# datavizweb/async-rl-tensorflow

Measured on AMD Instinct MI355X. Metric: env-steps/sec (whole node), Pong-v0 84×84×4, 1/2/4/8 MI355X + CPU ref, higher is better.
Workload: dtype fp32; 1 GPU; Pong-v0, 256 envs batched per MI355X, n-step=5, A3C conv net (nips trunk); frames=M1: raw RGB 210x160x3 + screen, game=Pong-v0, trunk=nips, head=feed-forward, env=device, envs_per_gpu=256, n_step=5, action_size=6, algo=a3c, parallelism=dp1, hipgraph=False

## Files before the change

async-rl-tensorflow_amd/csrc/gemm.h:

```cpp
#pragma once
#include "a3c_common.h"
#include "../../include/a3c_hip.h"



enum { EPI_STORE = 0, EPI_BIAS_RELU = 1, EPI_BIAS = 2, EPI_MASK = 3, EPI_MASKBITS = 4 };

struct GemmArgs {
  const float* A; int64_t lda;
  const float* B; int64_t ldb;
  float* C; int64_t ldc;
  int M, N, K;
  int epi;
  const float* bias;
  const float* mask; int64_t ldm;
  float* slab;
  int nsplit;
  int kchunk;
  float* colsum;
  int defer_reduce;
  int xcd;
  int max_wgs;
  int big;
  int wg_split;
  const uint32_t* maskbits;
};

int a3c_gemm(bool a_kcontig, bool b_ncontig, GemmArgs g, hipStream_t s, int* nsplit_eff = nullptr);
int a3c_gemm3(GemmArgs& g0, GemmArgs& g1, GemmArgs& g2, hipStream_t s);
int a3c_gemm_reduce(const GemmArgs& g, hipStream_t s);
int a3c_gemm_plan_split(int M, int N, int K, int target_blocks);

inline int a3c_gemm_effective_split(int K, int nsplit) {
  if (K < 1) return 1;
  int ktiles = (K + 15) / 16;
  if (nsplit < 1) nsplit = 1;
  int per = (ktiles + nsplit - 1) / nsplit;
  return (ktiles + per - 1) / per;
}
```

async-rl-tensorflow_amd/csrc/gemm.hip:

```cpp
#include <cstdlib>
#include "gemm.h"

#define BM 64
#define BN 64
#define BK 16
#define PAD 4

template <bool A_KC, bool B_NC>
__device__ inline void gemm_tile(const GemmArgs& g, int bx, int by, int bz, float (&As)[BK][BM + PAD],
                                 float (&Bs)[BK][BN + PAD]) {
  const int tid = threadIdx.x, lane = tid & 63, wid = tid >> 6;
  const int wm = wid >> 1, wn = wid & 1;
  const int m0 = by * BM, n0 = bx * BN;
  const int ks = bz;
  const int kbeg = ks * g.kchunk;
  const int kend = min(g.K, kbeg + g.kchunk);
  const bool do_colsum = g.colsum != nullptr && by == 0;

  int a_r, a_c, b_r, b_c;
  if (A_KC) { a_r = tid >> 2; a_c = (tid & 3) * 4; }
  else      { a_r = tid >> 4; a_c = (tid & 15) * 4; }
  if (B_NC) { b_r = tid >> 4; b_c = (tid & 15) * 4; }
  else      { b_r = tid >> 2; b_c = (tid & 3) * 4; }

  auto load_a = [&](int k0) -> f32x4 {
    f32x4 v = {0.f, 0.f, 0.f, 0.f};
    if (A_KC) {
      int m = m0 + a_r, k = k0 + a_c;
      if (m < g.M && k < kend) v = *(const f32x4*)(g.A + (int64_t)m * g.lda + k);
    } else {
      int k = k0 + a_r, m = m0 + a_c;
      if (k < kend && m < g.M) v = *(const f32x4*)(g.A + (int64_t)k * g.lda + m);
    }
    return v;
  };
  auto load_b = [&](int k0) -> f32x4 {
    f32x4 v = {0.f, 0.f, 0.f, 0.f};
    if (B_NC) {
      int k = k0 + b_r, n = n0 + b_c;
      if (k < kend && n < g.N) v = *(const f32x4*)(g.B + (int64_t)k * g.ldb + n);
    } else {
      int n = n0 + b_r, k = k0 + b_c;
      if (n < g.N && k < kend) v = *(const f32x4*)(g.B + (int64_t)n * g.ldb + k);
    }
    return v;
  };
  auto store_a = [&](f32x4 v) {
    if (A_KC) { As[a_c][a_r] = v[0]; As[a_c + 1][a_r] = v[1]; As[a_c + 2][a_r] = v[2]; As[a_c + 3][a_r] = v[3]; }
    else      { *(f32x4*)&As[a_r][a_c] = v; }
  };
  auto store_b = [&](f32x4 v) {
    if (B_NC) { *(f32x4*)&Bs[b_r][b_c] = v; }
    else      { Bs[b_c][b_r] = v[0]; Bs[b_c + 1][b_r] = v[1]; Bs[b_c + 2][b_r] = v[2]; Bs[b_c + 3][b_r] = v[3]; }
  };

  f32x16 acc = {};
  float csum = 0.f;
  f32x4 ra = load_a(kbeg), rb = load_b(kbeg);
  for (int k0 = kbeg; k0 < kend; k0 += BK) {
    __syncthreads();
    store_a(ra);
    store_b(rb);
    __syncthreads();
    if (k0 + BK < kend) { ra = load_a(k0 + BK); rb = load_b(k0 + BK); }
    if (do_colsum && tid < BN) {
#pragma unroll
      for (int k = 0; k < BK; ++k) csum += Bs[k][tid];
    }
    const int kh = lane >> 5, c = lane & 31;
#pragma unroll
    for (int kk = 0; kk < BK / 2; ++kk) {
      float a = As[2 * kk + kh][wm * 32 + c];
      float b = Bs[2 * kk + kh][wn * 32 + c];
      acc = __builtin_amdgcn_mfma_f32_32x32x2f32(a, b, acc, 0, 0, 0);
    }
  }

  const int col = n0 + wn * 32 + (lane & 31);
  if (g.nsplit > 1) {
    float* out = g.slab + (int64_t)ks * g.M * g.N;
#pragma unroll
    for (int r = 0; r < 16; ++r) {
      int row = m0 + wm * 32 + (r & 3) + 8 * (r >> 2) + 4 * (lane >> 5);
      if (row < g.M && col < g.N) ST_WT_G(out[(int64_t)row * g.N + col], acc[r]);
    }
  } else {
#pragma unroll
    for (int r = 0; r < 16; ++r) {
      int row = m0 + wm * 32 + (r & 3) + 8 * (r >> 2) + 4 * (lane >> 5);
      if (row < g.M && col < g.N) {
        float v = acc[r];
        if (g.epi == EPI_BIAS_RELU) v = fmaxf(v + g.bias[col], 0.f);
        else if (g.epi == EPI_BIAS) v = v + g.bias[col];
        else if (g.epi == EPI_MASK) v = g.mask[(int64_t)row * g.ldm + col] > 0.f ? v : 0.f;
#ifndef A3C_NO_MASKBITS
      else if (g.epi == EPI_MASKBITS) v = (g.maskbits[(int64_t)row * g.ldm + (col >> 5)] >> (col & 31)) & 1u ? v : 0.f;
#endif
        ST_WT_G(g.C[(int64_t)row * g.ldc + col], v);
      }
    }
  }
  if (do_colsum && tid < BN && n0 + tid < g.N) g.colsum[(int64_t)ks * g.N + n0 + tid] = csum;
}

template <bool A_KC, bool B_NC, int KS>
__global__ void __launch_bounds__(256 * KS) k_gemm_f32_wks(GemmArgs g) {
  WGLOG(5);
  __shared__ __attribute__((aligned(16))) float As[KS][BK][BM + PAD];
  __shared__ __attribute__((aligned(16))) float Bs[KS][BK][BN + PAD];
  const int grp = threadIdx.x >> 8, tid = threadIdx.x & 255, lane = tid & 63, wid = tid >> 6;
  const int wm = wid >> 1, wn = wid & 1;
  int bx = blockIdx.x, by = blockIdx.y;
  if (g.xcd == 1) {
    const int gx = (g.N + BN - 1) / BN, gy = (g.M + BM - 1) / BM;
    const int id = blockIdx.x, slot = id >> 3;
    by = 8 * (slot / gx) + (id & 7);
    bx = slot % gx;
    if (by >= gy) return;
  }
  const int m0 = by * BM, n0 = bx * BN;
  const int ktiles = (g.K + BK - 1) / BK, per = (ktiles + KS - 1) / KS;
  const int kbeg = grp * per * BK, kend = min(g.K, kbeg + per * BK);
  const bool do_colsum = g.colsum != nullptr && by == 0;
  int a_r, a_c, b_r, b_c;
  if (A_KC) { a_r = tid >> 2; a_c = (tid & 3) * 4; } else { a_r = tid >> 4; a_c = (tid & 15) * 4; }
  if (B_NC) { b_r = tid >> 4; b_c = (tid & 15) * 4; } else { b_r = tid >> 2; b_c = (tid & 3) * 4; }
  auto load_a = [&](int k0) -> f32x4 {
    f32x4 v = {0.f, 0.f, 0.f, 0.f};
    if (A_KC) {
      int m = m0 + a_r, k = k0 + a_c;
      if (m < g.M && k < kend) v = *(const f32x4*)(g.A + (int64_t)m * g.lda + k);
    } else {
      int k = k0 + a_r, m = m0 + a_c;
      if (k < kend && m < g.M) v = *(const f32x4*)(g.A + (int64_t)k * g.lda + m);
    }
    return v;
  };
  auto load_b = [&](int k0) -> f32x4 {
    f32x4 v = {0.f, 0.f, 0.f, 0.f};
    if (B_NC) {
      int k = k0 + b_r, n = n0 + b_c;
      if (k < kend && n < g.N) v = *(const f32x4*)(g.B + (int64_t)k * g.ldb + n);
    } else {
      int n = n0 + b_r, k = k0 + b_c;
      if (n < g.N && k < kend) v = *(const f32x4*)(g.B + (int64_t)n * g.ldb + k);
    }
    return v;
  };
  float (&as)[BK][BM + PAD] = As[grp];
  float (&bs)[BK][BN + PAD] = Bs[grp];
  f32x16 acc = {};
  float csum = 0.f;
  f32x4 ra = load_a(kbeg), rb = load_b(kbeg);
  for (int it = 0; it < per; ++it) {
    const int k0 = kbeg + it * BK;
    __syncthreads();
    if (A_KC) { as[a_c][a_r] = ra[0]; as[a_c + 1][a_r] = ra[1]; as[a_c + 2][a_r] = ra[2]; as[a_c + 3][a_r] = ra[3]; }
    else      { *(f32x4*)&as[a_r][a_c] = ra; }
    if (B_NC) { *(f32x4*)&bs[b_r][b_c] = rb; }
    else      { bs[b_c][b_r] = rb[0]; bs[b_c + 1][b_r] = rb[1]; bs[b_c + 2][b_r] = rb[2]; bs[b_c + 3][b_r] = rb[3]; }
    __syncthreads();
    if (it + 1 < per) { ra = load_a(k0 + BK); rb = load_b(k0 + BK); }
    if (do_colsum && tid < BN) {
#pragma unroll
      for (int k = 0; k < BK; ++k) csum += bs[k][tid];
    }
    const int kh = lane >> 5, c = lane & 31;
#pragma unroll
    for (int kk = 0; kk < BK / 2; ++kk)
      acc = __builtin_amdgcn_mfma_f32_32x32x2f32(as[2 * kk + kh][wm * 32 + c], bs[2 * kk + kh][wn * 32 + c], acc, 0, 0, 0);
  }
  static_assert(KS * BK * (BM + PAD) >= 16 * 256 + BN, "fold buffer");
  float* fold = &As[0][0][0];
  for (int q = 1; q < KS; ++q) {
    __syncthreads();
    if (grp == q) {
#pragma unroll
      for (int r = 0; r < 16; ++r) fold[r * 256 + tid] = acc[r];
      if (do_colsum && tid < BN) fold[16 * 256 + tid] = csum;
    }
    __syncthreads();
    if (grp == 0) {
#pragma unroll
      for (int r = 0; r < 16; ++r) acc[r] += fold[r * 256 + tid];
      if (do_colsum && tid < BN) csum += fold[16 * 256 + tid];
    }
  }
  if (grp != 0) return;
  const int col = n0 + wn * 32 + (lane & 31);
#pragma unroll
  for (int r = 0; r < 16; ++r) {
    const int row = m0 + wm * 32 + (r & 3) + 8 * (r >> 2) + 4 * (lane >> 5);
    if (row < g.M && col < g.N) {
      float v = acc[r];
      if (g.epi == EPI_BIAS_RELU) v = fmaxf(v + g.bias[col], 0.f);
      else if (g.epi == EPI_BIAS) v = v + g.bias[col];
      else if (g.epi == EPI_MASK) v = g.mask[(int64_t)row * g.ldm + col] > 0.f ? v : 0.f;
#ifndef A3C_NO_MASKBITS
      else if (g.epi == EPI_MASKBITS) v = (g.maskbits[(int64_t)row * g.ldm + (col >> 5)] >> (col & 31)) & 1u ? v : 0.f;
#endif
      ST_WT_G(g.C[(int64_t)row * g.ldc + col], v);
    }
  }
  if (do_colsum && tid < BN && n0 + tid < g.N) g.colsum[n0 + tid] = csum;
}

template <bool A_KC, bool B_NC>
__global__ void __launch_bounds__(256) k_gemm_f32_big(GemmArgs g) {
  WGLOG(5);
  constexpr int TM = 128, TN = 128;
  __shared__ __attribute__((aligned(16))) float As[BK][TM + PAD];
  __shared__ __attribute__((aligned(16))) float Bs[BK][TN + PAD];
  const int tid = threadIdx.x, lane = tid & 63, wid = tid >> 6;
  const int wm = wid >> 1, wn = wid & 1;
  const int m0 = blockIdx.y * TM, n0 = blockIdx.x * TN;
  const int ks = blockIdx.z;
  const int kbeg = ks * g.kchunk;
  const int kend = min(g.K, kbeg + g.kchunk);
  const bool do_colsum = g.colsum != nullptr && blockIdx.y == 0;
  auto a_rc = [&](int u, int& r, int& c) {
    if (A_KC) { r = (tid >> 2) + 64 * u; c = (tid & 3) * 4; }
    else      { r = (tid >> 5) + 8 * u; c = (tid & 31) * 4; }
  };
  auto b_rc = [&](int u, int& r, int& c) {
    if (B_NC) { r = (tid >> 5) + 8 * u; c = (tid & 31) * 4; }
    else      { r = (tid >> 2) + 64 * u; c = (tid & 3) * 4; }
  };
  auto load_a = [&](int k0, int u) -> f32x4 {
    f32x4 v = {0.f, 0.f, 0.f, 0.f};
    int r, c;
    a_rc(u, r, c);
    if (A_KC) {
      const int m = m0 + r, k = k0 + c;
      if (m < g.M && k < kend) v = *(const f32x4*)(g.A + (int64_t)m * g.lda + k);
    } else {
      const int k = k0 + r, m = m0 + c;
      if (k < kend && m < g.M) v = *(const f32x4*)(g.A + (int64_t)k * g.lda + m);
    }
    return v;
  };
  auto load_b = [&](int k0, int u) -> f32x4 {
    f32x4 v = {0.f, 0.f, 0.f, 0.f};
    int r, c;
    b_rc(u, r, c);
    if (B_NC) {
      const int k = k0 + r, n = n0 + c;
      if (k < kend && n < g.N) v = *(const f32x4*)(g.B + (int64_t)k * g.ldb + n);
    } else {
      const int n = n0 + r, k = k0 + c;
      if (n < g.N && k < kend) v = *(const f32x4*)(g.B + (int64_t)n * g.ldb + k);
    }
    return v;
  };
  auto store_a = [&](f32x4 v, int u) {
    int r, c;
    a_rc(u, r, c);
    if (A_KC) { As[c][r] = v[0]; As[c + 1][r] = v[1]; As[c + 2][r] = v[2]; As[c + 3][r] = v[3]; }
    else      { *(f32x4*)&As[r][c] = v; }
  };
  auto store_b = [&](f32x4 v, int u) {
    int r, c;
    b_rc(u, r, c);
    if (B_NC) { *(f32x4*)&Bs[r][c] = v; }
    else      { Bs[c][r] = v[0]; Bs[c + 1][r] = v[1]; Bs[c + 2][r] = v[2]; Bs[c + 3][r] = v[3]; }
  };
  f32x16 acc[2][2] = {};
  float csum = 0.f;
  f32x4 ra0 = load_a(kbeg, 0), ra1 = load_a(kbeg, 1), rb0 = load_b(kbeg, 0), rb1 = load_b(kbeg, 1);
  for (int k0 = kbeg; k0 < kend; k0 += BK) {
    __syncthreads();
    store_a(ra0, 0); store_a(ra1, 1);
    store_b(rb0, 0); store_b(rb1, 1);
    __syncthreads();
    if (k0 + BK < kend) {
      ra0 = load_a(k0 + BK, 0); ra1 = load_a(k0 + BK, 1);
      rb0 = load_b(k0 + BK, 0); rb1 = load_b(k0 + BK, 1);
    }
    if (do_colsum && tid < TN) {
#pragma unroll
      for (int k = 0; k < BK; ++k) csum += Bs[k][tid];
    }
    const int kh = lane >> 5, c = lane & 31;
#pragma unroll
    for (int kk = 0; kk < BK / 2; ++kk) {
      const float a0 = As[2 * kk + kh][wm * 64 + c], a1 = As[2 * kk + kh][wm * 64 + 32 + c];
      const float b0 = Bs[2 * kk + kh][wn * 64 + c], b1 = Bs[2 * kk + kh][wn * 64 + 32 + c];
      acc[0][0] = __builtin_amdgcn_mfma_f32_32x32x2f32(a0, b0, acc[0][0], 0, 0, 0);
      acc[0][1] = __builtin_amdgcn_mfma_f32_32x32x2f32(a0, b1, acc[0][1], 0, 0, 0);
      acc[1][0] = __builtin_amdgcn_mfma_f32_32x32x2f32(a1, b0, acc[1][0], 0, 0, 0);
      acc[1][1] = __builtin_amdgcn_mfma_f32_32x32x2f32(a1, b1, acc[1][1], 0, 0, 0);
    }
  }
#pragma unroll
  for (int i = 0; i < 2; ++i)
#pragma unroll
    for (int j = 0; j < 2; ++j) {
      const int col = n0 + wn * 64 + 32 * j + (lane & 31);
#pragma unroll
      for (int r = 0; r < 16; ++r) {
        const int row = m0 + wm * 64 + 32 * i + (r & 3) + 8 * (r >> 2) + 4 * (lane >> 5);
        if (row >= g.M || col >= g.N) continue;
        float v = acc[i][j][r];
        if (g.nsplit > 1) {
          ST_WT_G(g.slab[(int64_t)ks * g.M * g.N + (int64_t)row * g.N + col], v);
        } else {
          if (g.epi == EPI_BIAS_RELU) v = fmaxf(v + g.bias[col], 0.f);
          else if (g.epi == EPI_BIAS) v = v + g.bias[col];
          else if (g.epi == EPI_MASK) v = g.mask[(int64_t)row * g.ldm + col] > 0.f ? v : 0.f;
#ifndef A3C_NO_MASKBITS
      else if (g.epi == EPI_MASKBITS) v = (g.maskbits[(int64_t)row * g.ldm + (col >> 5)] >> (col & 31)) & 1u ? v : 0.f;
#endif
          ST_WT_G(g.C[(int64_t)row * g.ldc + col], v);
        }
      }
    }
  if (do_colsum && tid < TN && n0 + tid < g.N) g.colsum[(int64_t)ks * g.N + n0 + tid] = csum;
}

template <bool A_KC, bool B_NC>
__device__ inline void gemm_tile_id(const GemmArgs& g, int id, float (&As)[BK][BM + PAD], float (&Bs)[BK][BN + PAD]) {
  const int gx = (g.N + BN - 1) / BN, gy = (g.M + BM - 1) / BM;
  gemm_tile<A_KC, B_NC>(g, id % gx, (id / gx) % gy, id / (gx * gy), As, Bs);
}

template <bool A_KC, bool B_NC>
__global__ void __launch_bounds__(256) k_gemm_f32(GemmArgs g) {
  WGLOG(5);
  __shared__ __attribute__((aligned(16))) float As[BK][BM + PAD];
  __shared__ __attribute__((aligned(16))) float Bs[BK][BN + PAD];
  gemm_tile<A_KC, B_NC>(g, blockIdx.x, blockIdx.y, blockIdx.z, As, Bs);
}

template <bool A_KC, bool B_NC>
__global__ void __launch_bounds__(256) k_gemm_f32_x(GemmArgs g, int G, int J) {
  WGLOG(5);
  __shared__ __attribute__((aligned(16))) float As[BK][BM + PAD];
  __shared__ __attribute__((aligned(16))) float Bs[BK][BN + PAD];
  const int id = blockIdx.x, slot = id >> 3;
  const int grp = 8 * (slot / J) + (id & 7), j = slot % J;
  if (grp >= G) return;
  const int gx = (g.N + BN - 1) / BN, gy = (g.M + BM - 1) / BM;
  if (g.xcd == 1) gemm_tile<A_KC, B_NC>(g, j, grp % gy, grp / gy, As, Bs);
  else gemm_tile<A_KC, B_NC>(g, grp % gx, j, grp / gx, As, Bs);
}

template <bool A_KC, bool B_NC>
__global__ void __launch_bounds__(256) k_gemm_f32_p(GemmArgs g, int nb) {
  WGLOG(5);
  __shared__ __attribute__((aligned(16))) float As[BK][BM + PAD];
  __shared__ __attribute__((aligned(16))) float Bs[BK][BN + PAD];
  for (int id = blockIdx.x; id < nb; id += gridDim.x) gemm_tile_id<A_KC, B_NC>(g, id, As, Bs);
}

template <bool A_KC, bool B_NC>
__global__ void __launch_bounds__(256) k_gemm_f32_xp(GemmArgs g, int G, int J, int nid) {
  WGLOG(5);
  __shared__ __attribute__((aligned(16))) float As[BK][BM + PAD];
  __shared__ __attribute__((aligned(16))) float Bs[BK][BN + PAD];
  const int gx = (g.N + BN - 1) / BN, gy = (g.M + BM - 1) / BM;
  for (int id = blockIdx.x; id < nid; id += gridDim.x) {
    const int slot = id >> 3;
    const int grp = 8 * (slot / J) + (id & 7), j = slot % J;
    if (grp >= G) continue;
    if (g.xcd == 1) gemm_tile<A_KC, B_NC>(g, j, grp % gy, grp / gy, As, Bs);
    else gemm_tile<A_KC, B_NC>(g, grp % gx, j, grp / gx, As, Bs);
  }
}

__global__ void __launch_bounds__(256) k_gemm_multi(GemmArgs g0, GemmArgs g1, GemmArgs g2, int nb0, int nb1) {
  WGLOG(5);
  __shared__ __attribute__((aligned(16))) float As[BK][BM + PAD];
  __shared__ __attribute__((aligned(16))) float Bs[BK][BN + PAD];
  const int id = blockIdx.x;
  if (id < nb0) gemm_tile_id<false, true>(g0, id, As, Bs);
  else if (id < nb0 + nb1) gemm_tile_id<false, true>(g1, id - nb0, As, Bs);
  else gemm_tile_id<true, false>(g2, id - nb0 - nb1, As, Bs);
}

__global__ void k_reduce_slabs(const float* __restrict__ slab, int nsplit, int M, int N,
                               float* __restrict__ C, int64_t ldc, int epi,
                               const float* __restrict__ bias, const float* __restrict__ mask,
                               int64_t ldm, const uint32_t* __restrict__ maskbits) {
  WGLOG(8);
  int64_t i = (int64_t)blockIdx.x * blockDim.x + threadIdx.x;
  int64_t total = (int64_t)M * N;
  if (i >= total) return;
  float v = sum_strided(slab + i, nsplit, total);
  int row = (int)(i / N), col = (int)(i - (int64_t)row * N);
  if (epi == EPI_BIAS_RELU) v = fmaxf(v + bias[col], 0.f);
  else if (epi == EPI_BIAS) v = v + bias[col];
  else if (epi == EPI_MASK) v = mask[(int64_t)row * ldm + col] > 0.f ? v : 0.f;
#ifndef A3C_NO_MASKBITS
  else if (epi == EPI_MASKBITS) v = (maskbits[(int64_t)row * ldm + (col >> 5)] >> (col & 31)) & 1u ? v : 0.f;
#endif
  ST_WT_C(C[(int64_t)row * ldc + col], v);
}

int a3c_gemm_plan_split(int M, int N, int K, int target_blocks) {
  int tiles = ((M + BM - 1) / BM) * ((N + BN - 1) / BN);
  int ktiles = (K + BK - 1) / BK;
  int split = target_blocks / (tiles > 0 ? tiles : 1);
  if (split < 1) split = 1;
  if (split > ktiles) split = ktiles;
  if (split > 32) split = 32;
  return split;
}

static int gemm_setup(bool a_kc, bool b_nc, GemmArgs& g) {
  if (g.K < 1) return a3c_set_error(A3C_ERR_INVALID, "a3c_gemm", "K < 1");
  if (((a_kc || !b_nc) && (g.K & 3)) || (g.lda & 3) || (g.ldb & 3) ||
      (((uintptr_t)g.A | (uintptr_t)g.B) & 15) || (a_kc ? 0 : (g.M & 3)) || (b_nc ? (g.N & 3) : 0))
    return a3c_set_error(A3C_ERR_INVALID, "a3c_gemm", "unaligned operands (need 16-B alignment, dims %4)");
  if (g.nsplit < 1) g.nsplit = 1;
  const int ktiles = (g.K + BK - 1) / BK;
  const int per = (ktiles + g.nsplit - 1) / g.nsplit;
  g.kchunk = per * BK;
  g.nsplit = (ktiles + per - 1) / per;
  if (g.nsplit > 1 && !g.slab) return a3c_set_error(A3C_ERR_INVALID, "a3c_gemm", "split-K needs a slab");
  return 0;
}

static void gemm_reduce(const GemmArgs& g, hipStream_t s) {
  const int64_t total = (int64_t)g.M * g.N;
  hipLaunchKernelGGL(k_reduce_slabs, dim3((unsigned)((total + 255) / 256)), dim3(256), 0, s,
                     g.slab, g.nsplit, g.M, g.N, g.C, g.ldc, g.epi, g.bias, g.mask, g.ldm, g.maskbits);
}

int a3c_gemm3(GemmArgs& g0, GemmArgs& g1, GemmArgs& g2, hipStream_t s) {
  if (g0.M <= 0 || g0.N <= 0 || g1.M <= 0 || g1.N <= 0 || g2.M <= 0 || g2.N <= 0)
    return a3c_set_error(A3C_ERR_INVALID, "a3c_gemm3", "empty GEMM");
  int rc = gemm_setup(false, true, g0);
  if (!rc) rc = gemm_setup(false, true, g1);
  if (!rc) rc = gemm_setup(true, false, g2);
  if (rc) return rc;
  auto blocks = [](const GemmArgs& g) {
    return ((g.N + BN - 1) / BN) * ((g.M + BM - 1) / BM) * g.nsplit;
  };
  const int nb0 = blocks(g0), nb1 = blocks(g1), nb2 = blocks(g2);
  hipLaunchKernelGGL(k_gemm_multi, dim3((unsigned)(nb0 + nb1 + nb2)), dim3(256), 0, s, g0, g1, g2, nb0, nb1);
  A3C_CHECK(hipGetLastError());
  return 0;
}

int a3c_gemm_reduce(const GemmArgs& g, hipStream_t s) {
  if (g.nsplit > 1) {
    gemm_reduce(g, s);
    A3C_CHECK(hipGetLastError());
  }
  return 0;
}

int a3c_gemm(bool a_kc, bool b_nc, GemmArgs g, hipStream_t s, int* nsplit_eff) {
  if (g.M <= 0 || g.N <= 0) return 0;
  if (g.wg_split == 4) {
    g.nsplit = 1;
    int rc = gemm_setup(a_kc, b_nc, g);
    if (rc) return rc;
    if (nsplit_eff) *nsplit_eff = g.nsplit;
    const int gx = (g.N + BN - 1) / BN, gy = (g.M + BM - 1) / BM;
    const dim3 grid = g.xcd == 1 ? dim3((unsigned)(8 * ((gy + 7) / 8) * gx)) : dim3(gx, gy, 1);
    if (g.xcd != 0 && g.xcd != 1) return a3c_set_error(A3C_ERR_INVALID, "a3c_gemm", "wg_split: xcd 0 or 1");
    if (a_kc && b_nc) hipLaunchKernelGGL((k_gemm_f32_wks<true, true, 4>), grid, dim3(1024), 0, s, g);
    else if (a_kc && !b_nc) hipLaunchKernelGGL((k_gemm_f32_wks<true, false, 4>), grid, dim3(1024), 0, s, g);
    else if (!a_kc && b_nc) hipLaunchKernelGGL((k_gemm_f32_wks<false, true, 4>), grid, dim3(1024), 0, s, g);
    else hipLaunchKernelGGL((k_gemm_f32_wks<false, false, 4>), grid, dim3(1024), 0, s, g);
    A3C_CHECK(hipGetLastError());
    return 0;
  }
  if (g.wg_split > 1) return a3c_set_error(A3C_ERR_INVALID, "a3c_gemm", "wg_split: 4 only");
  int rc = gemm_setup(a_kc, b_nc, g);
  if (rc) return rc;
  if (nsplit_eff) *nsplit_eff = g.nsplit;
  dim3 grid((g.N + BN - 1) / BN, (g.M + BM - 1) / BM, g.nsplit);
  const int nb = (int)(grid.x * grid.y * grid.z);
  if (g.big) {
    const dim3 gb((g.N + 127) / 128, (g.M + 127) / 128, g.nsplit);
    if (a_kc && b_nc) hipLaunchKernelGGL((k_gemm_f32_big<true, true>), gb, dim3(256), 0, s, g);
    else if (a_kc && !b_nc) hipLaunchKernelGGL((k_gemm_f32_big<true, false>), gb, dim3(256), 0, s, g);
    else if (!a_kc && b_nc) hipLaunchKernelGGL((k_gemm_f32_big<false, true>), gb, dim3(256), 0, s, g);
    else hipLaunchKernelGGL((k_gemm_f32_big<false, false>), gb, dim3(256), 0, s, g);
    A3C_CHECK(hipGetLastError());
    return g.defer_reduce ? 0 : a3c_gemm_reduce(g, s);
  }
  if (g.xcd) {
    const int G = g.xcd == 1 ? (int)(grid.y * grid.z) : (int)(grid.x * grid.z);
    const int J = g.xcd == 1 ? (int)grid.x : (int)grid.y;
    const int nid = 8 * ((G + 7) / 8) * J;
    if (g.max_wgs > 0 && nid > g.max_wgs) {
      const dim3 gp((unsigned)(8 * ((g.max_wgs + 7) / 8)));
      if (a_kc && b_nc) hipLaunchKernelGGL((k_gemm_f32_xp<true, true>), gp, dim3(256), 0, s, g, G, J, nid);
      else if (a_kc && !b_nc) hipLaunchKernelGGL((k_gemm_f32_xp<true, false>), gp, dim3(256), 0, s, g, G, J, nid);
      else if (!a_kc && b_nc) hipLaunchKernelGGL((k_gemm_f32_xp<false, true>), gp, dim3(256), 0, s, g, G, J, nid);
      else hipLaunchKernelGGL((k_gemm_f32_xp<false, false>), gp, dim3(256), 0, s, g, G, J, nid);
      A3C_CHECK(hipGetLastError());
      return g.defer_reduce ? 0 : a3c_gemm_reduce(g, s);
    }
    const dim3 g1((unsigned)nid);
    if (a_kc && b_nc) hipLaunchKernelGGL((k_gemm_f32_x<true, true>), g1, dim3(256), 0, s, g, G, J);
    else if (a_kc && !b_nc) hipLaunchKernelGGL((k_gemm_f32_x<true, false>), g1, dim3(256), 0, s, g, G, J);
    else if (!a_kc && b_nc) hipLaunchKernelGGL((k_gemm_f32_x<false, true>), g1, dim3(256), 0, s, g, G, J);
    else hipLaunchKernelGGL((k_gemm_f32_x<false, false>), g1, dim3(256), 0, s, g, G, J);
    A3C_CHECK(hipGetLastError());
    return g.defer_reduce ? 0 : a3c_gemm_reduce(g, s);
  }
  if (g.max_wgs > 0 && nb > g.max_wgs) {
    const dim3 gp((unsigned)g.max_wgs);
    if (a_kc && b_nc) hipLaunchKernelGGL((k_gemm_f32_p<true, true>), gp, dim3(256), 0, s, g, nb);
    else if (a_kc && !b_nc) hipLaunchKernelGGL((k_gemm_f32_p<true, false>), gp, dim3(256), 0, s, g, nb);
    else if (!a_kc && b_nc) hipLaunchKernelGGL((k_gemm_f32_p<false, true>), gp, dim3(256), 0, s, g, nb);
    else hipLaunchKernelGGL((k_gemm_f32_p<false, false>), gp, dim3(256), 0, s, g, nb);
    A3C_CHECK(hipGetLastError());
    return g.defer_reduce ? 0 : a3c_gemm_reduce(g, s);
  }
  if (a_kc && b_nc) hipLaunchKernelGGL((k_gemm_f32<true, true>), grid, dim3(256), 0, s, g);
  else if (a_kc && !b_nc) hipLaunchKernelGGL((k_gemm_f32<true, false>), grid, dim3(256), 0, s, g);
  else if (!a_kc && b_nc) hipLaunchKernelGGL((k_gemm_f32<false, true>), grid, dim3(256), 0, s, g);
  else hipLaunchKernelGGL((k_gemm_f32<false, false>), grid, dim3(256), 0, s, g);
  A3C_CHECK(hipGetLastError());
  return g.defer_reduce ? 0 : a3c_gemm_reduce(g, s);
}

static int64_t slab_bytes(int M, int N, int split) {
  return split > 1 ? (int64_t)split * M * N * (int64_t)sizeof(float) : 0;
}

static int gemm_desc_args(const char* what, const a3c_gemm_desc* d, void* ws, int64_t ws_bytes, GemmArgs& g) {
  auto bad = [&](const char* why) { return a3c_set_error(A3C_ERR_INVALID, what, why); };
  auto mis = [](const void* p, uintptr_t a) { return ((uintptr_t)p & (a - 1)) != 0; };
  if (!d) return bad("desc is NULL");
  if (!d->A || !d->B || !d->C) return bad("A, B or C is NULL");
  if (d->M < 1 || d->N < 1) return bad("M < 1 or N < 1");
  if (d->K < 1) return bad("K < 1");
  if (d->nsplit < 1) return bad("nsplit < 1");
  if (d->epi < A3C_GEMM_STORE || d->epi > A3C_GEMM_MASKBITS) return bad("unknown epi");
  if ((d->epi == A3C_GEMM_BIAS_RELU || d->epi == A3C_GEMM_BIAS) && !d->bias) return bad("epi needs bias");
  if (d->epi == A3C_GEMM_MASK && !d->mask) return bad("epi needs mask");
  if (d->epi == A3C_GEMM_MASKBITS && !d->maskbits) return bad("epi needs maskbits");
  if (d->wg_split != 0 && d->wg_split != 4) return bad("wg_split: 0 or 4");
  if (d->xcd < 0 || d->xcd > 2) return bad("xcd: 0, 1 or 2");
  if (d->wg_split && d->xcd == 2) return bad("wg_split: xcd 0 or 1");
  if (d->max_wgs < 0) return bad("max_wgs < 0");
  const bool akc = d->a_kcontig != 0, bnc = d->b_ncontig != 0;
  if (mis(d->A, 16) || mis(d->B, 16)) return bad("A and B need 16-byte alignment");
  if (mis(d->C, 4) || mis(d->bias, 4) || mis(d->mask, 4) || mis(d->maskbits, 4) || mis(d->colsum, 4))
    return bad("C, bias, mask, maskbits, colsum need 4-byte alignment");
  if ((d->lda & 3) || (d->ldb & 3)) return bad("lda and ldb must be multiples of 4");
  if ((akc || !bnc) && (d->K & 3)) return bad("K must be a multiple of 4 in this layout");
  if (!akc && (d->M & 3)) return bad("M must be a multiple of 4 when a is k-strided");
  if (bnc && (d->N & 3)) return bad("N must be a multiple of 4 when b is n-contiguous");
  if (d->lda < (akc ? d->K : d->M) || d->ldb < (bnc ? d->N : d->K) || d->ldc < d->N)
    return bad("lda, ldb or ldc shorter than a row");
  if (d->epi == A3C_GEMM_MASK && d->ldm < d->N) return bad("ldm shorter than a mask row");
  if (d->epi == A3C_GEMM_MASKBITS && d->ldm < (d->N + 31) / 32) return bad("ldm shorter than a row of mask words");
  const int eff = d->wg_split ? 1 : a3c_gemm_effective_split(d->K, d->nsplit);
  if (eff > 1) {
    if (!ws) return bad("split-K needs a workspace");
    if (mis(ws, 16)) return bad("workspace needs 16-byte alignment");
    if (ws_bytes < slab_bytes(d->M, d->N, eff)) return bad("workspace too small (a3c_gemm_workspace_bytes)");
  }
  g = GemmArgs{};
  g.A = d->A; g.lda = d->lda; g.B = d->B; g.ldb = d->ldb; g.C = d->C; g.ldc = d->ldc;
  g.M = d->M; g.N = d->N; g.K = d->K;
  g.epi = d->epi; g.bias = d->bias; g.mask = d->mask; g.maskbits = d->maskbits; g.ldm = d->ldm;
  g.slab = eff > 1 ? (float*)ws : nullptr;
  g.nsplit = d->nsplit; g.colsum = d->colsum;
  g.xcd = d->xcd; g.max_wgs = d->max_wgs; g.big = d->big ? 1 : 0; g.wg_split = d->wg_split;
  return 0;
}

extern "C" int a3c_gemm_workspace_bytes(int M, int N, int K, int nsplit, int* nsplit_eff, int64_t* bytes) {
  if (M < 1 || N < 1 || K < 1 || nsplit < 1)
    return a3c_set_error(A3C_ERR_INVALID, "a3c_gemm_workspace_bytes", "M, N, K or nsplit < 1");
  const int eff = a3c_gemm_effective_split(K, nsplit);
  if (nsplit_eff) *nsplit_eff = eff;
  if (bytes) *bytes = slab_bytes(M, N, eff);
  return 0;
}

extern "C" int a3c_gemm_f32(const a3c_gemm_desc* d, void* workspace, int64_t workspace_bytes, int* nsplit_eff,
                            void* stream) {
  GemmArgs g;
  if (int rc = gemm_desc_args("a3c_gemm_f32", d, workspace, workspace_bytes, g)) return rc;
  return a3c_gemm(d->a_kcontig != 0, d->b_ncontig != 0, g, (hipStream_t)stream, nsplit_eff);
}

extern "C" int a3c_gemm3_f32(const a3c_gemm_desc* d, void* const* workspaces, const int64_t* workspace_bytes,
                             int* nsplit_eff, void* stream) {
  const char* what = "a3c_gemm3_f32";
  if (!d) return a3c_set_error(A3C_ERR_INVALID, what, "desc is NULL");
  GemmArgs g[3];
  for (int i = 0; i < 3; ++i) {
    if ((d[i].a_kcontig != 0) != (i == 2) || (d[i].b_ncontig != 0) != (i < 2))
      return a3c_set_error(A3C_ERR_INVALID, what, "layouts: d[0], d[1] (a k-strided, b n-contiguous), d[2] (k, k)");
    if (d[i].wg_split || d[i].big || d[i].xcd || d[i].max_wgs)
      return a3c_set_error(A3C_ERR_INVALID, what, "wg_split, big, xcd and max_wgs must be 0");
    if (int rc = gemm_desc_args(what, d + i, workspaces ? workspaces[i] : nullptr,
                                workspace_bytes ? workspace_bytes[i] : 0, g[i]))
      return rc;
  }
  hipStream_t s = (hipStream_t)stream;
  if (int rc = a3c_gemm3(g[0], g[1], g[2], s)) return rc;
  for (int i = 0; i < 3; ++i) {
    if (nsplit_eff) nsplit_eff[i] = g[i].nsplit;
    if (int rc = a3c_gemm_reduce(g[i], s)) return rc;
  }
  return 0;
}

#ifdef A3C_WGLOG
WGLOG_BIND(a3c_wglog_bind_gemm)
#endif
```

Before: 4.996 million env-steps/s.

## Unify fp32 GEMM mainloop with double-buffered LDS, swizzled layout and vector fragments

Replaces the three separate GEMM inner loops with a shared templated mainloop. It uses two LDS stages with a register prefetch two k-tiles ahead and one barrier per k-tile instead of two, so global loads overlap the MFMA work. K-contiguous operands go into an XOR-swizzled LDS image so fragments load as f32x4 vectors instead of scalar LDS reads. Launch bounds gain occupancy hints, at the cost of doubled LDS per block and more register pressure, and the index/out-of-bounds handling becomes more intricate.

```diff
diff --git a/async-rl-tensorflow_amd/csrc/gemm.h b/async-rl-tensorflow_amd/csrc/gemm.h
--- a/async-rl-tensorflow_amd/csrc/gemm.h
+++ b/async-rl-tensorflow_amd/csrc/gemm.h
@@ -5,6 +5,16 @@
 
 
 enum { EPI_STORE = 0, EPI_BIAS_RELU = 1, EPI_BIAS = 2, EPI_MASK = 3, EPI_MASKBITS = 4 };
+
+constexpr int GEMM_BK = 16, GEMM_PREFETCH = 2, GEMM_STAGES = 2;
+
+__host__ __device__ constexpr int gemm_kpos(int k) { return (k & 1) * 8 + (k >> 1); }
+__host__ __device__ constexpr int gemm_img_off(int row, int pos) {
+  return row * 16 + ((((pos >> 2) ^ (row >> 2)) & 3) << 2) + (pos & 3);
+}
+__host__ __device__ constexpr int gemm_img_floats(bool kcontig, int rows) {
+  return kcontig ? rows * GEMM_BK : GEMM_BK * (rows + 4);
+}
 
 struct GemmArgs {
   const float* A; int64_t lda;
diff --git a/async-rl-tensorflow_amd/csrc/gemm.hip b/async-rl-tensorflow_amd/csrc/gemm.hip
--- a/async-rl-tensorflow_amd/csrc/gemm.hip
+++ b/async-rl-tensorflow_amd/csrc/gemm.hip
@@ -3,12 +3,141 @@
 
 #define BM 64
 #define BN 64
-#define BK 16
+#define BK GEMM_BK
 #define PAD 4
 
-template <bool A_KC, bool B_NC>
-__device__ inline void gemm_tile(const GemmArgs& g, int bx, int by, int bz, float (&As)[BK][BM + PAD],
-                                 float (&Bs)[BK][BN + PAD]) {
+typedef float f32x2 __attribute__((ext_vector_type(2)));
+template <int V> struct IntC { static constexpr int value = V; };
+
+template <bool KC, int R>
+struct GemmOperand {
+  static constexpr int U = R / 64;
+  static constexpr int LD = R + PAD;
+  static constexpr int FLOATS = gemm_img_floats(KC, R);
+  const float* p[U];
+  const float* base;
+  int64_t kstep;
+  int kq[U], so[U];
+  bool ok[U];
+
+  __device__ void init(const float* X, int64_t ld, int x0, int xn, int tid) {
+#pragma unroll
+    for (int u = 0; u < U; ++u) {
+      int r, k;
+      if (KC) { r = (tid >> 2) + 64 * u; k = (tid & 3) * 4; p[u] = X + (int64_t)(x0 + r) * ld + k; so[u] = gemm_img_off(r, k >> 1); }
+      else    { k = tid / (R / 4) + (1024 / R) * u; r = (tid % (R / 4)) * 4; p[u] = X + (int64_t)k * ld + x0 + r; so[u] = k * LD + r; }
+      ok[u] = x0 + r < xn;
+      kq[u] = k;
+    }
+    kstep = KC ? 1 : ld;
+    base = X;
+  }
+  __device__ bool inside(int u, int k0, int kend) const { return ok[u] && k0 + kq[u] < kend; }
+  __device__ f32x4 load(int u, int k0, bool in) const {
+    return *(const f32x4*)(in ? p[u] + (int64_t)k0 * kstep : base);
+  }
+  __device__ void store(float* img, int u, f32x4 v, bool in) const {
+    if (!in) v = f32x4{0.f, 0.f, 0.f, 0.f};
+    if (KC) {
+      *(f32x2*)(img + so[u]) = f32x2{v[0], v[2]};
+      *(f32x2*)(img + (so[u] ^ 8)) = f32x2{v[1], v[3]};
+    } else {
+      *(f32x4*)(img + so[u]) = v;
+    }
+  }
+  __device__ static f32x4 frag(const float* img, int row, int kh, int g) {
+    if (KC) return *(const f32x4*)(img + gemm_img_off(row, kh * 8 + g * 4));
+    f32x4 v;
+#pragma unroll
+    for (int i = 0; i < 4; ++i) v[i] = img[(2 * (4 * g + i) + kh) * LD + row];
+    return v;
+  }
+  __device__ static float at(const float* img, int k, int row) {
+    return KC ? img[gemm_img_off(row, gemm_kpos(k))] : img[k * LD + row];
+  }
+};
+
+template <bool A_KC, bool B_NC, int TM, int TN>
+__device__ inline void gemm_mainloop(const GemmArgs& g, int m0, int n0, int kbeg, int kend, int ntiles,
+                                     bool do_colsum, int tid, float* As, float* Bs,
+                                     f32x16 (&acc)[TM / 64][TN / 64], float& csum) {
+  using OA = GemmOperand<A_KC, TM>;
+  using OB = GemmOperand<!B_NC, TN>;
+  constexpr int MI = TM / 64, NI = TN / 64;
+  const int lane = tid & 63, wid = tid >> 6;
+  const int kh = lane >> 5;
+  const int arow = (wid >> 1) * (TM / 2) + (lane & 31), brow = (wid & 1) * (TN / 2) + (lane & 31);
+  OA oa;
+  OB ob;
+  oa.init(g.A, g.lda, m0, g.M, tid);
+  ob.init(g.B, g.ldb, n0, g.N, tid);
+  f32x4 ga[2][MI], gb[2][NI];
+  bool ia[2][MI], ib[2][NI];
+  f32x4 fa[2][MI], fb[2][NI];
+  auto gload = [&](auto S, int k0) {
+    constexpr int s = decltype(S)::value;
+#pragma unroll
+    for (int u = 0; u < MI; ++u) { ia[s][u] = oa.inside(u, k0, kend); ga[s][u] = oa.load(u, k0, ia[s][u]); }
+#pragma unroll
+    for (int u = 0; u < NI; ++u) { ib[s][u] = ob.inside(u, k0, kend); gb[s][u] = ob.load(u, k0, ib[s][u]); }
+  };
+  auto stage = [&](auto S, float* a, float* b) {
+    constexpr int s = decltype(S)::value;
+#pragma unroll
+    for (int u = 0; u < MI; ++u) oa.store(a, u, ga[s][u], ia[s][u]);
+#pragma unroll
+    for (int u = 0; u < NI; ++u) ob.store(b, u, gb[s][u], ib[s][u]);
+  };
+  auto frags = [&](auto G, const float* a, const float* b) {
+    constexpr int gi = decltype(G)::value;
+#pragma unroll
+    for (int i = 0; i < MI; ++i) fa[gi][i] = OA::frag(a, arow + 32 * i, kh, gi);
+#pragma unroll
+    for (int j = 0; j < NI; ++j) fb[gi][j] = OB::frag(b, brow + 32 * j, kh, gi);
+  };
+  auto mfmas = [&](auto G) {
+    constexpr int gi = decltype(G)::value;
+#pragma unroll
+    for (int e = 0; e < 4; ++e)
+#pragma unroll
+      for (int i = 0; i < MI; ++i)
+#pragma unroll
+        for (int j = 0; j < NI; ++j)
+          acc[i][j] = __builtin_amdgcn_mfma_f32_32x32x2f32(fa[gi][i][e], fb[gi][j][e], acc[i][j], 0, 0, 0);
+  };
+  auto step = [&](auto PC, int t) {
+    constexpr int P = decltype(PC)::value;
+    float* a = As + P * OA::FLOATS;
+    float* b = Bs + P * OB::FLOATS;
+    float* an = As + (P ^ 1) * OA::FLOATS;
+    float* bn = Bs + (P ^ 1) * OB::FLOATS;
+    frags(IntC<1>{}, a, b);
+    if (do_colsum && tid < TN) {
+#pragma unroll
+      for (int k = 0; k < BK; ++k) csum += OB::at(b, k, tid);
+    }
+    mfmas(IntC<0>{});
+    if (t + 1 < ntiles) stage(IntC<P ^ 1>{}, an, bn);
+    gload(IntC<P ^ 1>{}, kbeg + (t + 1 + GEMM_PREFETCH) * BK);
+    __syncthreads();
+    if (t + 1 < ntiles) frags(IntC<0>{}, an, bn);
+    mfmas(IntC<1>{});
+  };
+  __syncthreads();
+  gload(IntC<0>{}, kbeg);
+  gload(IntC<1>{}, kbeg + BK);
+  stage(IntC<0>{}, As, Bs);
+  gload(IntC<0>{}, kbeg + 2 * BK);
+  __syncthreads();
+  frags(IntC<0>{}, As, Bs);
+  for (int t = 0; t < ntiles; t += 2) {
+    step(IntC<0>{}, t);
+    if (t + 1 < ntiles) step(IntC<1>{}, t + 1);
+  }
+}
+
+template <bool A_KC, bool B_NC>
+__device__ inline void gemm_tile(const GemmArgs& g, int bx, int by, int bz, float* As, float* Bs) {
   const int tid = threadIdx.x, lane = tid & 63, wid = tid >> 6;
   const int wm = wid >> 1, wn = wid & 1;
   const int m0 = by * BM, n0 = bx * BN;
@@ -16,65 +145,10 @@
   const int kbeg = ks * g.kchunk;
   const int kend = min(g.K, kbeg + g.kchunk);
   const bool do_colsum = g.colsum != nullptr && by == 0;
-
-  int a_r, a_c, b_r, b_c;
-  if (A_KC) { a_r = tid >> 2; a_c = (tid & 3) * 4; }
-  else      { a_r = tid >> 4; a_c = (tid & 15) * 4; }
-  if (B_NC) { b_r = tid >> 4; b_c = (tid & 15) * 4; }
-  else      { b_r = tid >> 2; b_c = (tid & 3) * 4; }
-
-  auto load_a = [&](int k0) -> f32x4 {
-    f32x4 v = {0.f, 0.f, 0.f, 0.f};
-    if (A_KC) {
-      int m = m0 + a_r, k = k0 + a_c;
-      if (m < g.M && k < kend) v = *(const f32x4*)(g.A + (int64_t)m * g.lda + k);
-    } else {
-      int k = k0 + a_r, m = m0 + a_c;
-      if (k < kend && m < g.M) v = *(const f32x4*)(g.A + (int64_t)k * g.lda + m);
-    }
-    return v;
-  };
-  auto load_b = [&](int k0) -> f32x4 {
-    f32x4 v = {0.f, 0.f, 0.f, 0.f};
-    if (B_NC) {
-      int k = k0 + b_r, n = n0 + b_c;
-      if (k < kend && n < g.N) v = *(const f32x4*)(g.B + (int64_t)k * g.ldb + n);
-    } else {
-      int n = n0 + b_r, k = k0 + b_c;
-      if (n < g.N && k < kend) v = *(const f32x4*)(g.B + (int64_t)n * g.ldb + k);
-    }
-    return v;
-  };
-  auto store_a = [&](f32x4 v) {
-    if (A_KC) { As[a_c][a_r] = v[0]; As[a_c + 1][a_r] = v[1]; As[a_c + 2][a_r] = v[2]; As[a_c + 3][a_r] = v[3]; }
-    else      { *(f32x4*)&As[a_r][a_c] = v; }
-  };
-  auto store_b = [&](f32x4 v) {
-    if (B_NC) { *(f32x4*)&Bs[b_r][b_c] = v; }
-    else      { Bs[b_c][b_r] = v[0]; Bs[b_c + 1][b_r] = v[1]; Bs[b_c + 2][b_r] = v[2]; Bs[b_c + 3][b_r] = v[3]; }
-  };
-
-  f32x16 acc = {};
+  f32x16 accs[1][1] = {};
   float csum = 0.f;
-  f32x4 ra = load_a(kbeg), rb = load_b(kbeg);
-  for (int k0 = kbeg; k0 < kend; k0 += BK) {
-    __syncthreads();
-    store_a(ra);
-    store_b(rb);
-    __syncthreads();
-    if (k0 + BK < kend) { ra = load_a(k0 + BK); rb = load_b(k0 + BK); }
-    if (do_colsum && tid < BN) {
-#pragma unroll
-      for (int k = 0; k < BK; ++k) csum += Bs[k][tid];
-    }
-    const int kh = lane >> 5, c = lane & 31;
-#pragma unroll
-    for (int kk = 0; kk < BK / 2; ++kk) {
-      float a = As[2 * kk + kh][wm * 32 + c];
-      float b = Bs[2 * kk + kh][wn * 32 + c];
-      acc = __builtin_amdgcn_mfma_f32_32x32x2f32(a, b, acc, 0, 0, 0);
-    }
-  }
+  gemm_mainloop<A_KC, B_NC, BM, BN>(g, m0, n0, kbeg, kend, (kend - kbeg + BK - 1) / BK, do_colsum, tid, As, Bs, accs, csum);
+  const f32x16 acc = accs[0][0];
 
   const int col = n0 + wn * 32 + (lane & 31);
   if (g.nsplit > 1) {
@@ -106,8 +180,9 @@
 template <bool A_KC, bool B_NC, int KS>
 __global__ void __launch_bounds__(256 * KS) k_gemm_f32_wks(GemmArgs g) {
   WGLOG(5);
-  __shared__ __attribute__((aligned(16))) float As[KS][BK][BM + PAD];
-  __shared__ __attribute__((aligned(16))) float Bs[KS][BK][BN + PAD];
+  constexpr int A_FLOATS = GEMM_STAGES * gemm_img_floats(A_KC, BM), B_FLOATS = GEMM_STAGES * gemm_img_floats(!B_NC, BN);
+  __shared__ __attribute__((aligned(16))) float As[KS * A_FLOATS];
+  __shared__ __attribute__((aligned(16))) float Bs[KS * B_FLOATS];
   const int grp = threadIdx.x >> 8, tid = threadIdx.x & 255, lane = tid & 63, wid = tid >> 6;
   const int wm = wid >> 1, wn = wid & 1;
   int bx = blockIdx.x, by = blockIdx.y;
@@ -122,56 +197,13 @@
   const int ktiles = (g.K + BK - 1) / BK, per = (ktiles + KS - 1) / KS;
   const int kbeg = grp * per * BK, kend = min(g.K, kbeg + per * BK);
   const bool do_colsum = g.colsum != nullptr && by == 0;
-  int a_r, a_c, b_r, b_c;
-  if (A_KC) { a_r = tid >> 2; a_c = (tid & 3) * 4; } else { a_r = tid >> 4; a_c = (tid & 15) * 4; }
-  if (B_NC) { b_r = tid >> 4; b_c = (tid & 15) * 4; } else { b_r = tid >> 2; b_c = (tid & 3) * 4; }
-  auto load_a = [&](int k0) -> f32x4 {
-    f32x4 v = {0.f, 0.f, 0.f, 0.f};
-    if (A_KC) {
-      int m = m0 + a_r, k = k0 + a_c;
-      if (m < g.M && k < kend) v = *(const f32x4*)(g.A + (int64_t)m * g.lda + k);
-    } else {
-      int k = k0 + a_r, m = m0 + a_c;
-      if (k < kend && m < g.M) v = *(const f32x4*)(g.A + (int64_t)k * g.lda + m);
-    }
-    return v;
-  };
-  auto load_b = [&](int k0) -> f32x4 {
-    f32x4 v = {0.f, 0.f, 0.f, 0.f};
-    if (B_NC) {
-      int k = k0 + b_r, n = n0 + b_c;
-      if (k < kend && n < g.N) v = *(const f32x4*)(g.B + (int64_t)k * g.ldb + n);
-    } else {
-      int n = n0 + b_r, k = k0 + b_c;
-      if (n < g.N && k < kend) v = *(const f32x4*)(g.B + (int64_t)n * g.ldb + k);
-    }
-    return v;
-  };
-  float (&as)[BK][BM + PAD] = As[grp];
-  float (&bs)[BK][BN + PAD] = Bs[grp];
-  f32x16 acc = {};
+  f32x16 accs[1][1] = {};
   float csum = 0.f;
-  f32x4 ra = load_a(kbeg), rb = load_b(kbeg);
-  for (int it = 0; it < per; ++it) {
-    const int k0 = kbeg + it * BK;
-    __syncthreads();
-    if (A_KC) { as[a_c][a_r] = ra[0]; as[a_c + 1][a_r] = ra[1]; as[a_c + 2][a_r] = ra[2]; as[a_c + 3][a_r] = ra[3]; }
-    else      { *(f32x4*)&as[a_r][a_c] = ra; }
-    if (B_NC) { *(f32x4*)&bs[b_r][b_c] = rb; }
-    else      { bs[b_c][b_r] = rb[0]; bs[b_c + 1][b_r] = rb[1]; bs[b_c + 2][b_r] = rb[2]; bs[b_c + 3][b_r] = rb[3]; }
-    __syncthreads();
-    if (it + 1 < per) { ra = load_a(k0 + BK); rb = load_b(k0 + BK); }
-    if (do_colsum && tid < BN) {
-#pragma unroll
-      for (int k = 0; k < BK; ++k) csum += bs[k][tid];
-    }
-    const int kh = lane >> 5, c = lane & 31;
-#pragma unroll
-    for (int kk = 0; kk < BK / 2; ++kk)
-      acc = __builtin_amdgcn_mfma_f32_32x32x2f32(as[2 * kk + kh][wm * 32 + c], bs[2 * kk + kh][wn * 32 + c], acc, 0, 0, 0);
-  }
-  static_assert(KS * BK * (BM + PAD) >= 16 * 256 + BN, "fold buffer");
-  float* fold = &As[0][0][0];
+  gemm_mainloop<A_KC, B_NC, BM, BN>(g, m0, n0, kbeg, kend, per, do_colsum, tid, As + grp * A_FLOATS, Bs + grp * B_FLOATS,
+                                    accs, csum);
+  f32x16 acc = accs[0][0];
+  static_assert(KS * A_FLOATS >= 16 * 256 + BN, "fold buffer");
+  float* fold = As;
   for (int q = 1; q < KS; ++q) {
     __syncthreads();
     if (grp == q) {
@@ -206,11 +238,11 @@
 }
 
 template <bool A_KC, bool B_NC>
-__global__ void __launch_bounds__(256) k_gemm_f32_big(GemmArgs g) {
+__global__ void __launch_bounds__(256, 2) k_gemm_f32_big(GemmArgs g) {
   WGLOG(5);
   constexpr int TM = 128, TN = 128;
-  __shared__ __attribute__((aligned(16))) float As[BK][TM + PAD];
-  __shared__ __attribute__((aligned(16))) float Bs[BK][TN + PAD];
+  __shared__ __attribute__((aligned(16))) float As[GEMM_STAGES * gemm_img_floats(A_KC, TM)];
+  __shared__ __attribute__((aligned(16))) float Bs[GEMM_STAGES * gemm_img_floats(!B_NC, TN)];
   const int tid = threadIdx.x, lane = tid & 63, wid = tid >> 6;
   const int wm = wid >> 1, wn = wid & 1;
   const int m0 = blockIdx.y * TM, n0 = blockIdx.x * TN;
@@ -218,79 +250,9 @@
   const int kbeg = ks * g.kchunk;
   const int kend = min(g.K, kbeg + g.kchunk);
   const bool do_colsum = g.colsum != nullptr && blockIdx.y == 0;
-  auto a_rc = [&](int u, int& r, int& c) {
-    if (A_KC) { r = (tid >> 2) + 64 * u; c = (tid & 3) * 4; }
-    else      { r = (tid >> 5) + 8 * u; c = (tid & 31) * 4; }
-  };
-  auto b_rc = [&](int u, int& r, int& c) {
-    if (B_NC) { r = (tid >> 5) + 8 * u; c = (tid & 31) * 4; }
-    else      { r = (tid >> 2) + 64 * u; c = (tid & 3) * 4; }
-  };
-  auto load_a = [&](int k0, int u) -> f32x4 {
-    f32x4 v = {0.f, 0.f, 0.f, 0.f};
-    int r, c;
-    a_rc(u, r, c);
-    if (A_KC) {
-      const int m = m0 + r, k = k0 + c;
-      if (m < g.M && k < kend) v = *(const f32x4*)(g.A + (int64_t)m * g.lda + k);
-    } else {
-      const int k = k0 + r, m = m0 + c;
-      if (k < kend && m < g.M) v = *(const f32x4*)(g.A + (int64_t)k * g.lda + m);
-    }
-    return v;
-  };
-  auto load_b = [&](int k0, int u) -> f32x4 {
-    f32x4 v = {0.f, 0.f, 0.f, 0.f};
-    int r, c;
-    b_rc(u, r, c);
-    if (B_NC) {
-      const int k = k0 + r, n = n0 + c;
-      if (k < kend && n < g.N) v = *(const f32x4*)(g.B + (int64_t)k * g.ldb + n);
-    } else {
-      const int n = n0 + r, k = k0 + c;
-      if (n < g.N && k < kend) v = *(const f32x4*)(g.B + (int64_t)n * g.ldb + k);
-    }
-    return v;
-  };
-  auto store_a = [&](f32x4 v, int u) {
-    int r, c;
-    a_rc(u, r, c);
-    if (A_KC) { As[c][r] = v[0]; As[c + 1][r] = v[1]; As[c + 2][r] = v[2]; As[c + 3][r] = v[3]; }
-    else      { *(f32x4*)&As[r][c] = v; }
-  };
-  auto store_b = [&](f32x4 v, int u) {
-    int r, c;
-    b_rc(u, r, c);
-    if (B_NC) { *(f32x4*)&Bs[r][c] = v; }
-    else      { Bs[c][r] = v[0]; Bs[c + 1][r] = v[1]; Bs[c + 2][r] = v[2]; Bs[c + 3][r] = v[3]; }
-  };
   f32x16 acc[2][2] = {};
   float csum = 0.f;
-  f32x4 ra0 = load_a(kbeg, 0), ra1 = load_a(kbeg, 1), rb0 = load_b(kbeg, 0), rb1 = load_b(kbeg, 1);
-  for (int k0 = kbeg; k0 < kend; k0 += BK) {
-    __syncthreads();
-    store_a(ra0, 0); store_a(ra1, 1);
-    store_b(rb0, 0); store_b(rb1, 1);
-    __syncthreads();
-    if (k0 + BK < kend) {
-      ra0 = load_a(k0 + BK, 0); ra1 = load_a(k0 + BK, 1);
-      rb0 = load_b(k0 + BK, 0); rb1 = load_b(k0 + BK, 1);
-    }
-    if (do_colsum && tid < TN) {
-#pragma unroll
-      for (int k = 0; k < BK; ++k) csum += Bs[k][tid];
-    }
-    const int kh = lane >> 5, c = lane & 31;
-#pragma unroll
-    for (int kk = 0; kk < BK / 2; ++kk) {
-      const float a0 = As[2 * kk + kh][wm * 64 + c], a1 = As[2 * kk + kh][wm * 64 + 32 + c];
-      const float b0 = Bs[2 * kk + kh][wn * 64 + c], b1 = Bs[2 * kk + kh][wn * 64 + 32 + c];
-      acc[0][0] = __builtin_amdgcn_mfma_f32_32x32x2f32(a0, b0, acc[0][0], 0, 0, 0);
-      acc[0][1] = __builtin_amdgcn_mfma_f32_32x32x2f32(a0, b1, acc[0][1], 0, 0, 0);
-      acc[1][0] = __builtin_amdgcn_mfma_f32_32x32x2f32(a1, b0, acc[1][0], 0, 0, 0);
-      acc[1][1] = __builtin_amdgcn_mfma_f32_32x32x2f32(a1, b1, acc[1][1], 0, 0, 0);
-    }
-  }
+  gemm_mainloop<A_KC, B_NC, TM, TN>(g, m0, n0, kbeg, kend, (kend - kbeg + BK - 1) / BK, do_colsum, tid, As, Bs, acc, csum);
 #pragma unroll
   for (int i = 0; i < 2; ++i)
 #pragma unroll
@@ -318,24 +280,24 @@
 }
 
 template <bool A_KC, bool B_NC>
-__device__ inline void gemm_tile_id(const GemmArgs& g, int id, float (&As)[BK][BM + PAD], float (&Bs)[BK][BN + PAD]) {
+__device__ inline void gemm_tile_id(const GemmArgs& g, int id, float* As, float* Bs) {
   const int gx = (g.N + BN - 1) / BN, gy = (g.M + BM - 1) / BM;
   gemm_tile<A_KC, B_NC>(g, id % gx, (id / gx) % gy, id / (gx * gy), As, Bs);
 }
 
 template <bool A_KC, bool B_NC>
-__global__ void __launch_bounds__(256) k_gemm_f32(GemmArgs g) {
-  WGLOG(5);
-  __shared__ __attribute__((aligned(16))) float As[BK][BM + PAD];
-  __shared__ __attribute__((aligned(16))) float Bs[BK][BN + PAD];
+__global__ void __launch_bounds__(256, 4) k_gemm_f32(GemmArgs g) {
+  WGLOG(5);
+  __shared__ __attribute__((aligned(16))) float As[GEMM_STAGES * gemm_img_floats(A_KC, BM)];
+  __shared__ __attribute__((aligned(16))) float Bs[GEMM_STAGES * gemm_img_floats(!B_NC, BN)];
   gemm_tile<A_KC, B_NC>(g, blockIdx.x, blockIdx.y, blockIdx.z, As, Bs);
 }
 
 template <bool A_KC, bool B_NC>
-__global__ void __launch_bounds__(256) k_gemm_f32_x(GemmArgs g, int G, int J) {
-  WGLOG(5);
-  __shared__ __attribute__((aligned(16))) float As[BK][BM + PAD];
-  __shared__ __attribute__((aligned(16))) float Bs[BK][BN + PAD];
+__global__ void __launch_bounds__(256, 4) k_gemm_f32_x(GemmArgs g, int G, int J) {
+  WGLOG(5);
+  __shared__ __attribute__((aligned(16))) float As[GEMM_STAGES * gemm_img_floats(A_KC, BM)];
+  __shared__ __attribute__((aligned(16))) float Bs[GEMM_STAGES * gemm_img_floats(!B_NC, BN)];
   const int id = blockIdx.x, slot = id >> 3;
   const int grp = 8 * (slot / J) + (id & 7), j = slot % J;
   if (grp >= G) return;
@@ -345,18 +307,18 @@
 }
 
 template <bool A_KC, bool B_NC>
-__global__ void __launch_bounds__(256) k_gemm_f32_p(GemmArgs g, int nb) {
-  WGLOG(5);
-  __shared__ __attribute__((aligned(16))) float As[BK][BM + PAD];
-  __shared__ __attribute__((aligned(16))) float Bs[BK][BN + PAD];
+__global__ void __launch_bounds__(256, 4) k_gemm_f32_p(GemmArgs g, int nb) {
+  WGLOG(5);
+  __shared__ __attribute__((aligned(16))) float As[GEMM_STAGES * gemm_img_floats(A_KC, BM)];
+  __shared__ __attribute__((aligned(16))) float Bs[GEMM_STAGES * gemm_img_floats(!B_NC, BN)];
   for (int id = blockIdx.x; id < nb; id += gridDim.x) gemm_tile_id<A_KC, B_NC>(g, id, As, Bs);
 }
 
 template <bool A_KC, bool B_NC>
-__global__ void __launch_bounds__(256) k_gemm_f32_xp(GemmArgs g, int G, int J, int nid) {
-  WGLOG(5);
-  __shared__ __attribute__((aligned(16))) float As[BK][BM + PAD];
-  __shared__ __attribute__((aligned(16))) float Bs[BK][BN + PAD];
+__global__ void __launch_bounds__(256, 4) k_gemm_f32_xp(GemmArgs g, int G, int J, int nid) {
+  WGLOG(5);
+  __shared__ __attribute__((aligned(16))) float As[GEMM_STAGES * gemm_img_floats(A_KC, BM)];
+  __shared__ __attribute__((aligned(16))) float Bs[GEMM_STAGES * gemm_img_floats(!B_NC, BN)];
   const int gx = (g.N + BN - 1) / BN, gy = (g.M + BM - 1) / BM;
   for (int id = blockIdx.x; id < nid; id += gridDim.x) {
     const int slot = id >> 3;
@@ -367,10 +329,11 @@
   }
 }
 
-__global__ void __launch_bounds__(256) k_gemm_multi(GemmArgs g0, GemmArgs g1, GemmArgs g2, int nb0, int nb1) {
-  WGLOG(5);
-  __shared__ __attribute__((aligned(16))) float As[BK][BM + PAD];
-  __shared__ __attribute__((aligned(16))) float Bs[BK][BN + PAD];
+__global__ void __launch_bounds__(256, 4) k_gemm_multi(GemmArgs g0, GemmArgs g1, GemmArgs g2, int nb0, int nb1) {
+  WGLOG(5);
+  static_assert(gemm_img_floats(false, BM) >= gemm_img_floats(true, BM), "k_gemm_multi LDS");
+  __shared__ __attribute__((aligned(16))) float As[GEMM_STAGES * gemm_img_floats(false, BM)];
+  __shared__ __attribute__((aligned(16))) float Bs[GEMM_STAGES * gemm_img_floats(false, BN)];
   const int id = blockIdx.x;
   if (id < nb0) gemm_tile_id<false, true>(g0, id, As, Bs);
   else if (id < nb0 + nb1) gemm_tile_id<false, true>(g1, id - nb0, As, Bs);
```

Result: slower. 4.311 million env-steps/s (-13.7%).
